# pyani-plus/pyani-plus

Measured on AMD Instinct MI355X. Metric: pairwise genome comparisons/sec (N x N ANI matrix), higher is better.
Workload: dtype u64

## Files before the change

### pyani_plus_amd/csrc/kmer_hash.hip

```cpp
#include <cstdlib>
#include <type_traits>
#include <utility>

#include "pa_internal.h"
#include "murmur_dev.h"

namespace {

using namespace pa_dev;

constexpr int kThreads = 256;
constexpr uint32_t kStageCap = 1024;

constexpr int pow2_floor(int k) { int c = 1; while (2 * c <= k) c *= 2; return c; }

__device__ __forceinline__ uint32_t find_genome(const uint32_t *__restrict__ genome_blk, uint32_t n, uint32_t blk) {
  uint32_t lo = 0, hi = n;
  while (hi - lo > 1) {
    uint32_t mid = (lo + hi) >> 1;
    if (genome_blk[mid] <= blk) lo = mid; else hi = mid;
  }
  return lo;
}

__device__ __forceinline__ void region_append(const CandSink &s, uint32_t g, uint64_t h) {
  const uint64_t slot = atomicAdd(&s.cursor[g], 1u);
  if (slot < s.region_off[g + 1] - s.region_off[g]) s.cand_hash[s.region_off[g] + slot] = h; else *s.overflow = 1u;
}

__device__ __forceinline__ void append_candidate(const CandSink &s, uint32_t g, uint64_t h) {
  if (s.region_off) {
    region_append(s, g, h);
  } else {
    const unsigned long long slot = atomicAdd(reinterpret_cast<unsigned long long *>(s.count), 1ULL);
    if (slot < s.cap) {
      s.cand_hash[slot] = h;
      s.cand_genome[slot] = g;
    }
  }
}

__device__ __forceinline__ void stage_candidate(const CandSink &s, uint64_t (&s_hash)[kStageCap], uint32_t (&s_blk)[kStageCap],
                                                uint32_t &s_n, uint32_t t, uint64_t h) {
  const uint32_t slot = atomicAdd(&s_n, 1u);
  if (slot < kStageCap) {
    s_hash[slot] = h;
    s_blk[slot] = t;
  } else if (s.region_off) {
    region_append(s, find_genome(s.genome_blk, s.n_genomes, t), h);
  } else {
    const unsigned long long g = atomicAdd(reinterpret_cast<unsigned long long *>(s.count), 1ULL);
    if (g < s.cap) {
      s.cand_hash[g] = h;
      s.cand_genome[g] = find_genome(s.genome_blk, s.n_genomes, t);
    }
  }
}

__device__ __forceinline__ void flush_staged(const CandSink &s, const uint64_t (&s_hash)[kStageCap], const uint32_t (&s_blk)[kStageCap],
                                             const uint32_t &s_n, unsigned long long &s_base, uint32_t blk0, uint32_t n_blocks64) {
  const uint32_t tid = threadIdx.x;
  __syncthreads();
  const uint32_t n = min(s_n, kStageCap);
  if (n == 0) return;
  if (s.region_off) {
    const uint32_t b0 = blk0 + blockIdx.x * kThreads;
    const uint32_t b1 = min(b0 + (uint32_t)kThreads, n_blocks64) - 1u;
    const uint32_t g0 = find_genome(s.genome_blk, s.n_genomes, b0);
    if (s.genome_blk[g0 + 1] > b1) {
      if (tid == 0) s_base = atomicAdd(&s.cursor[g0], n);
      __syncthreads();
      const uint64_t room = s.region_off[g0 + 1] - s.region_off[g0];
      uint64_t *__restrict__ dst = s.cand_hash + s.region_off[g0];
      for (uint32_t i = tid; i < n; i += kThreads) {
        const uint64_t slot = s_base + i;
        if (slot < room) dst[slot] = s_hash[i]; else *s.overflow = 1u;
      }
    } else {
      for (uint32_t i = tid; i < n; i += kThreads)
        region_append(s, find_genome(s.genome_blk, s.n_genomes, s_blk[i]), s_hash[i]);
    }
    return;
  }
  if (tid == 0) s_base = atomicAdd(reinterpret_cast<unsigned long long *>(s.count), (unsigned long long)n);
  __syncthreads();
  const unsigned long long base = s_base;
  for (uint32_t i = tid; i < n; i += kThreads) {
    const unsigned long long g = base + i;
    if (g < s.cap) {
      s.cand_hash[g] = s_hash[i];
      s.cand_genome[g] = find_genome(s.genome_blk, s.n_genomes, s_blk[i]);
    }
  }
}

__device__ __forceinline__ uint32_t rev_groups32(uint32_t x) {
  x = __builtin_bitreverse32(x);
  return ((x >> 1) & 0x55555555u) | ((x & 0x55555555u) << 1);
}

template <int K, bool LUT>
__global__ __launch_bounds__(kThreads) void kmer_hash_kernel(
    const uint4 *__restrict__ packed, const uint2 *__restrict__ mask, const uint64_t *__restrict__ dirty, uint32_t n_blocks64,
    const uint32_t *__restrict__ genome_blk, uint32_t n_genomes, uint64_t max_hash,
    uint64_t *__restrict__ cand_hash, uint32_t *__restrict__ cand_genome, uint64_t cap,
    unsigned long long *__restrict__ count, const uint64_t *__restrict__ region_off, uint32_t *__restrict__ cursor,
    uint32_t *__restrict__ overflow, uint32_t blk0) {
  static_assert(K >= 1 && K <= 32, "a k-mer is one 64-bit register pair");
  __shared__ uint64_t s_hash[kStageCap];
  __shared__ uint32_t s_blk[kStageCap];
  __shared__ uint32_t s_n;
  __shared__ unsigned long long s_base;
  constexpr int kWords = (K + 7) / 8;
  __shared__ uint64_t s_lo[LUT ? kWords : 1][256];
  __shared__ uint32_t s_hi[LUT ? kWords : 1][256];

  const uint32_t tid = threadIdx.x;
  const CandSink sink{cand_hash, cand_genome, cap, reinterpret_cast<uint64_t *>(count), region_off, cursor, overflow, genome_blk, n_genomes};
  const uint32_t max_hi = (uint32_t)(max_hash >> 32);
  const bool take_all = max_hi == 0xffffffffu;
  const uint32_t screen_hi = max_hi + 1u;
  if (tid == 0) s_n = 0;
  if constexpr (LUT) fill_first_products(s_lo, s_hi, tid, std::integral_constant<int, K>{});
  __syncthreads();

  const uint32_t t = blk0 + blockIdx.x * kThreads + tid;
  if (t < n_blocks64) {
    const uint4 cur = packed[t];
    uint2 pw = make_uint2(0u, 0u);
    if (t > 0) pw = reinterpret_cast<const uint2 *>(packed)[2 * (uint64_t)t - 1];
    uint32_t d1 = 0u, d2 = 0u;
    const uint32_t wave_blk = __builtin_amdgcn_readfirstlane(t & ~63u);
    const uint64_t dirty_word = dirty[wave_blk >> 6];
    if ((dirty_word >> (t & 63u)) & 1ull) {
      const uint2 m = mask[t];
      uint32_t d0 = t > 0 ? mask[t - 1].y : 0xffffffffu;
      d1 = m.x;
      d2 = m.y;
      int c = 1;
#pragma unroll
      for (; 2 * c <= K; c *= 2) {
        d2 |= alignbit(d2, d1, 32 - c);
        d1 |= alignbit(d1, d0, 32 - c);
        d0 |= d0 << c;
      }
      constexpr int cc = pow2_floor(K);
      constexpr int r = K - cc;
      if constexpr (r > 0) {
        d2 |= alignbit(d2, d1, 32 - r);
        d1 |= alignbit(d1, d0, 32 - r);
      }
    }
    const uint32_t bad[2] = {d1, d2};
    if ((d1 & d2) != 0xffffffffu) {
      constexpr uint64_t kMask = (K == 32) ? ~0ULL : ((1ULL << (2 * K)) - 1);
      constexpr uint32_t kMaskHi = (uint32_t)(kMask >> 32);
      uint32_t fw[8] = {pw.x, pw.y, cur.x, cur.y, cur.z, cur.w, 0u, 0u};
      uint32_t rw[6];
#pragma unroll
      for (int j = 0; j < 6; ++j) rw[j] = ~rev_groups32(fw[5 - j]);
      auto columns = [&](auto base_tag, int i_begin, int i_end) {
        constexpr int kBase = decltype(base_tag)::value;
#pragma unroll 1
        for (int i = i_begin; i < i_end; ++i) {
          constexpr int kOff = 33 - K;
          const uint32_t fo = 2u * (uint32_t)((i + kOff) & 15), ro = 30u - 2u * (uint32_t)i;
          uint32_t A[5], B[5];
#pragma unroll
          for (int j = 0; j < 5; ++j) {
            A[j] = alignbit(fw[kBase + j + 1], fw[kBase + j], fo);
            B[j] = alignbit(rw[j + 1], rw[j], ro);
          }
#pragma unroll
          for (int wi = 0; wi < 4; ++wi) {
            const uint32_t f_lo = A[wi], f_hi = A[wi + 1], r_lo = B[3 - wi], r_hi = B[4 - wi];
          const uint64_t f_lsb = u64_of(f_lo, f_hi) & kMask, r_lsb = u64_of(r_lo, r_hi) & kMask;
          const uint64_t fwd = __builtin_amdgcn_uicmpl(f_lsb, r_lsb, 37 );
          uint32_t clo, chi;
          asm("s_nop 1\n\tv_cndmask_b32_e64 %0, %1, %2, %3" : "=v"(clo) : "v"((uint32_t)r_lsb), "v"((uint32_t)f_lsb), "s"(fwd));
          asm("v_cndmask_b32_e64 %0, %1, %2, %3" : "=v"(chi) : "v"((uint32_t)(r_lsb >> 32)), "v"((uint32_t)(f_lsb >> 32)), "s"(fwd), "v"(clo));
          uint64_t P[4] = {0, 0, 0, 0};
#pragma unroll
          for (int j = 0; j < kWords; ++j) {
            const uint32_t src = j < 2 ? clo : chi;
            if constexpr (LUT) {
              P[j] = first_product(s_lo, s_hi, j, src);
            } else {
              const uint32_t glo = (src >> (16 * (j & 1))) & 0xffu, ghi = (src >> (16 * (j & 1) + 8)) & 0xffu;
              const uint64_t word = u64_of(ascii_group(glo, K - 8 * j), ascii_group(ghi, K - 8 * j - 4));
              P[j] = word * ((j & 1) ? kC2 : kC1);
            }
          }
          (void)kMaskHi;
          uint64_t U, V;
          murmur3_pre_last_mul<K>(P, U, V);
          if (passes_screen(U, V, take_all, screen_hi)) {
            const uint64_t h = last_mul_and_fold(U, V);
            if (h > max_hash || ((bad[wi >> 1] >> (16 * (wi & 1) + i)) & 1u)) continue;
            stage_candidate(sink, s_hash, s_blk, s_n, t, h);
          }
          }
        }
      };
      constexpr int kOff0 = 33 - K, kSplit = (kOff0 & 15) ? 16 - (kOff0 & 15) : 16;
      columns(std::integral_constant<int, (kOff0 >> 4)>{}, 0, kSplit);
      if constexpr (kSplit < 16) columns(std::integral_constant<int, (kOff0 >> 4) + 1>{}, kSplit, 16);
    }
  }
  flush_staged(sink, s_hash, s_blk, s_n, s_base, blk0, n_blocks64);
}

template <int K>
__global__ __launch_bounds__(kThreads) void kmer_hash_wide_kernel(
    const uint4 *__restrict__ packed, const uint2 *__restrict__ mask, const uint64_t *__restrict__ dirty, uint32_t n_blocks64,
    const uint32_t *__restrict__ genome_blk, uint32_t n_genomes, uint64_t max_hash,
    uint64_t *__restrict__ cand_hash, uint32_t *__restrict__ cand_genome, uint64_t cap,
    unsigned long long *__restrict__ count, const uint64_t *__restrict__ region_off, uint32_t *__restrict__ cursor,
    uint32_t *__restrict__ overflow, uint32_t blk0) {
  static_assert(K >= 33 && K <= 64, "k-mers of 65 to 128 bits");
  __shared__ uint64_t s_hash[kStageCap];
  __shared__ uint32_t s_blk[kStageCap];
  __shared__ uint32_t s_n;
  __shared__ unsigned long long s_base;
  constexpr int kWords = (K + 7) / 8;
  __shared__ uint64_t s_lo[kWords][256];
  __shared__ uint32_t s_hi[kWords][256];
  const uint32_t tid = threadIdx.x;
  const CandSink sink{cand_hash, cand_genome, cap, reinterpret_cast<uint64_t *>(count), region_off, cursor, overflow, genome_blk, n_genomes};
  const uint32_t max_hi = (uint32_t)(max_hash >> 32);
  const bool take_all = max_hi == 0xffffffffu;
  const uint32_t screen_hi = max_hi + 1u;
  if (tid == 0) s_n = 0;
  fill_first_products(s_lo, s_hi, tid, std::integral_constant<int, K>{});
  __syncthreads();

  const uint32_t t = blk0 + blockIdx.x * kThreads + tid;
  if (t < n_blocks64) {
    const uint4 cur = packed[t];
    const uint4 prev = t > 0 ? packed[t - 1] : make_uint4(0u, 0u, 0u, 0u);
    uint32_t d2 = 0u, d3 = 0u;
    const uint32_t wave_blk = __builtin_amdgcn_readfirstlane(t & ~63u);
    const uint64_t dirty_word = dirty[wave_blk >> 6];
    const uint64_t before = wave_blk ? dirty[(wave_blk >> 6) - 1] >> 63 : 1ull;
    const uint64_t dirty_or_prev = dirty_word | (dirty_word << 1) | before;
    if ((dirty_or_prev >> (t & 63u)) & 1ull) {
      const uint2 m = mask[t];
      uint32_t d0 = 0xffffffffu, d1 = 0xffffffffu;
      if (t > 0) { const uint2 mp = mask[t - 1]; d0 = mp.x; d1 = mp.y; }
      d2 = m.x;
      d3 = m.y;
#pragma unroll
      for (int c = 1; c <= 16; c *= 2) {
        d3 |= alignbit(d3, d2, 32 - c);
        d2 |= alignbit(d2, d1, 32 - c);
        d1 |= alignbit(d1, d0, 32 - c);
        d0 |= d0 << c;
      }
      if constexpr (K == 64) {
        d3 |= d2; d2 |= d1; d1 |= d0;
      } else {
        constexpr int r = K - 32;
        d3 |= alignbit(d3, d2, 32 - r);
        d2 |= alignbit(d2, d1, 32 - r);
        d1 |= alignbit(d1, d0, 32 - r);
      }
    }
    const uint32_t bad[2] = {d2, d3};
    if ((d2 & d3) != 0xffffffffu) {
      constexpr uint32_t kMask2 = (2 * K - 64 >= 32) ? 0xffffffffu : ((1u << (2 * K - 64)) - 1u);
      constexpr uint32_t kMask3 = (2 * K - 96 >= 32) ? 0xffffffffu : (2 * K - 96 <= 0 ? 0u : ((1u << ((2 * K - 96) & 31)) - 1u));
      const uint32_t fw[10] = {prev.x, prev.y, prev.z, prev.w, cur.x, cur.y, cur.z, cur.w, 0u, 0u};
      uint32_t rw[10];
#pragma unroll
      for (int j = 0; j < 10; ++j) rw[j] = ~rev_groups32(fw[9 - j]);
      auto columns = [&](auto base_tag, int i_begin, int i_end) {
        constexpr int kBase = decltype(base_tag)::value;
#pragma unroll 1
        for (int i = i_begin; i < i_end; ++i) {
          constexpr int kOff = 65 - K;
          const uint32_t fo = 2u * (uint32_t)((i + kOff) & 15), ro = 30u - 2u * (uint32_t)i;
          uint32_t A[7], B[7];
#pragma unroll
          for (int j = 0; j < 7; ++j) {
            A[j] = alignbit(fw[kBase + j + 1], fw[kBase + j], fo);
            B[j] = alignbit(rw[j + 3], rw[j + 2], ro);
          }
#pragma unroll
          for (int wi = 0; wi < 4; ++wi) {
            const uint32_t f0 = A[wi], f1 = A[wi + 1], f2 = A[wi + 2] & kMask2, f3 = A[wi + 3] & kMask3;
            const uint32_t r0 = B[3 - wi], r1 = B[4 - wi], r2 = B[5 - wi] & kMask2, r3 = B[6 - wi] & kMask3;
            const uint64_t lt_hi = __builtin_amdgcn_uicmpl(u64_of(f2, f3), u64_of(r2, r3), 36 );
            const uint64_t eq_hi = __builtin_amdgcn_uicmpl(u64_of(f2, f3), u64_of(r2, r3), 32 );
            const uint64_t le_lo = __builtin_amdgcn_uicmpl(u64_of(f0, f1), u64_of(r0, r1), 37 );
            const uint64_t fwd = lt_hi | (eq_hi & le_lo);
            uint32_t c0, c1, c2, c3;
            asm("s_nop 1\n\tv_cndmask_b32_e64 %0, %1, %2, %3" : "=v"(c0) : "v"(r0), "v"(f0), "s"(fwd));
            asm("v_cndmask_b32_e64 %0, %1, %2, %3" : "=v"(c1) : "v"(r1), "v"(f1), "s"(fwd), "v"(c0));
            asm("v_cndmask_b32_e64 %0, %1, %2, %3" : "=v"(c2) : "v"(r2), "v"(f2), "s"(fwd), "v"(c1));
            asm("v_cndmask_b32_e64 %0, %1, %2, %3" : "=v"(c3) : "v"(r3), "v"(f3), "s"(fwd), "v"(c2));
            const uint32_t cw[4] = {c0, c1, c2, c3};
            uint64_t P[8] = {0, 0, 0, 0, 0, 0, 0, 0};
#pragma unroll
            for (int j = 0; j < kWords; ++j) P[j] = first_product(s_lo, s_hi, j, cw[j >> 1]);
            uint64_t U, V;
            murmur3_pre_last_mul<K>(P, U, V);
            if (passes_screen(U, V, take_all, screen_hi)) {
              const uint64_t h = last_mul_and_fold(U, V);
              if (h > max_hash || ((bad[wi >> 1] >> (16 * (wi & 1) + i)) & 1u)) continue;
              stage_candidate(sink, s_hash, s_blk, s_n, t, h);
            }
          }
        }
      };
      constexpr int kOff0 = 65 - K, kSplit = (kOff0 & 15) ? 16 - (kOff0 & 15) : 16;
      columns(std::integral_constant<int, (kOff0 >> 4)>{}, 0, kSplit);
      if constexpr (kSplit < 16) columns(std::integral_constant<int, (kOff0 >> 4) + 1>{}, kSplit, 16);
    }
  }
  flush_staged(sink, s_hash, s_blk, s_n, s_base, blk0, n_blocks64);
}

constexpr int kLongIter = 32;
__global__ __launch_bounds__(kThreads) void kmer_hash_long_kernel(
    const uint32_t *__restrict__ packed, const uint32_t *__restrict__ mask, uint64_t pos0, uint64_t pos1, uint32_t k,
    const uint32_t *__restrict__ genome_blk, uint32_t n_genomes, uint64_t max_hash, uint64_t *__restrict__ cand_hash,
    uint32_t *__restrict__ cand_genome, uint64_t cap, unsigned long long *__restrict__ count,
    const uint64_t *__restrict__ region_off, uint32_t *__restrict__ cursor, uint32_t *__restrict__ overflow) {
  __shared__ uint64_t s_lo[8][256];
  __shared__ uint32_t s_hi[8][256];
  const uint32_t tid = threadIdx.x;
  const CandSink sink{cand_hash, cand_genome, cap, reinterpret_cast<uint64_t *>(count), region_off, cursor, overflow, genome_blk, n_genomes};
  const uint32_t n_words = (k + 7u) >> 3;
  const uint32_t max_hi = (uint32_t)(max_hash >> 32);
  const bool take_all = max_hi == 0xffffffffu;
  const uint32_t screen_hi = max_hi + 1u;
  fill_first_products(s_lo, s_hi, tid, k);
  __syncthreads();
  const uint64_t wg_first = pos0 + ((uint64_t)blockIdx.y * gridDim.x + blockIdx.x) * (uint64_t)(kThreads * kLongIter);
#pragma unroll 1
  for (int it = 0; it < kLongIter; ++it) {
  const uint64_t e = wg_first + (uint64_t)it * kThreads + tid;
  if (e >= pos1 || e + 1 < k) continue;
  const uint64_t a = e + 1 - k;
  {
    const uint64_t m0 = a >> 5, m_last = e >> 5;
    const uint32_t sm = (uint32_t)(a & 31u);
    const uint32_t w0 = mask[m0], w1 = m0 + 1 <= m_last ? mask[m0 + 1] : 0u, w2 = m0 + 2 <= m_last ? mask[m0 + 2] : 0u;
    const uint32_t b0 = alignbit(w1, w0, sm), b1 = alignbit(w2, w1, sm);
    const uint32_t top = k == 64 ? 0xffffffffu : ((1u << (k - 32u)) - 1u);
    if (b0 | (b1 & top)) continue;
  }
  uint32_t F[4], R[4];
  {
    const uint64_t p0 = a >> 4, p_last = e >> 4;
    const uint32_t sp = 2u * (uint32_t)(a & 15u);
    uint32_t w[5];
#pragma unroll
    for (int i = 0; i < 5; ++i) w[i] = p0 + i <= p_last ? packed[p0 + i] : 0u;
#pragma unroll
    for (int i = 0; i < 4; ++i) F[i] = alignbit(w[i + 1], w[i], sp);
    const uint32_t used = 2u * k - 64u;
    if (used < 32u) { F[2] &= (1u << used) - 1u; F[3] = 0u; }
    else if (used < 64u) F[3] &= (1u << (used - 32u)) - 1u;
    const uint32_t C[6] = {~rev_groups32(F[3]), ~rev_groups32(F[2]), ~rev_groups32(F[1]), ~rev_groups32(F[0]), 0u, 0u};
    const uint32_t s = 128u - 2u * k, ws = s >> 5, bs = s & 31u;
#pragma unroll
    for (int i = 0; i < 4; ++i) R[i] = ws ? alignbit(C[i + 2], C[i + 1], bs) : alignbit(C[i + 1], C[i], bs);
    if (used < 32u) { R[2] &= (1u << used) - 1u; R[3] = 0u; }
    else if (used < 64u) R[3] &= (1u << (used - 32u)) - 1u;
  }
  const uint64_t f_hi = u64_of(F[2], F[3]), f_lo = u64_of(F[0], F[1]), r_hi = u64_of(R[2], R[3]), r_lo = u64_of(R[0], R[1]);
  const bool fwd = f_hi < r_hi || (f_hi == r_hi && f_lo <= r_lo);
  uint32_t c[4];
#pragma unroll
  for (int i = 0; i < 4; ++i) c[i] = fwd ? F[i] : R[i];
  uint64_t P[8] = {0, 0, 0, 0, 0, 0, 0, 0};
#pragma unroll
  for (uint32_t j = 0; j < 8; ++j) {
    if (j >= n_words) break;
    P[j] = first_product(s_lo, s_hi, j, c[j >> 1]);
  }
  uint64_t U, V;
  murmur3_pre_last_mul_rt(P, k, U, V);
  if (!passes_screen(U, V, take_all, screen_hi)) continue;
  const uint64_t h = last_mul_and_fold(U, V);
  if (h > max_hash) continue;
  append_candidate(sink, find_genome(genome_blk, n_genomes, (uint32_t)(e >> 6)), h);
  }
}

template <class Kernel>
int launch_blocks(pa_ctx *c, const char *name, Kernel kernel, const KmerHashArgs &a) {
  const ArenaView &v = a.arena;
  const CandSink &s = a.sink;
  return pa_launch(c, name, kernel, false, ceil_div(v.n_blocks64 - a.blk0, kThreads), kThreads, 0, a.stream,
                   reinterpret_cast<const uint4 *>(v.packed), reinterpret_cast<const uint2 *>(v.mask), v.dirty,
                   (uint32_t)v.n_blocks64, s.genome_blk, s.n_genomes, a.max_hash, s.cand_hash, s.cand_genome, s.cap,
                   reinterpret_cast<unsigned long long *>(s.count), s.region_off, s.cursor, s.overflow, (uint32_t)a.blk0);
}

template <int K>
int launch_k(pa_ctx *c, const KmerHashArgs &a) {
  if constexpr (K > 32) {
    return launch_blocks(c, "kmer_hash_wide_kernel", kmer_hash_wide_kernel<K>, a);
  } else {
    if constexpr (K == 31) {
      static const bool arithmetic = [] {
        const char *v = PA_TOOL_ENV("PA_KMER_VARIANT");
        return v && v[0] == '0';
      }();
      if (arithmetic) return launch_blocks(c, "kmer_hash_kernel<31, false>", kmer_hash_kernel<K, false>, a);
    }
    return launch_blocks(c, "kmer_hash_kernel", kmer_hash_kernel<K, true>, a);
  }
}

}

int pa_launch_kmer_hash(pa_ctx *c, const KmerHashArgs &a) {
  const uint64_t n_blocks64 = a.arena.n_blocks64;
  PA_REQUIRE(n_blocks64 < (1ULL << 32), "arena too large: %llu blocks of 64 bases", (unsigned long long)n_blocks64);
  if (n_blocks64 <= a.blk0) return PA_OK;
  const char *long_form = PA_TOOL_ENV("PA_KMER_LONG");
  if (a.k > 32 && a.k <= 64 && long_form && long_form[0] == 'p') {
    const CandSink &s = a.sink;
    const uint64_t pos0 = a.blk0 * 64, pos1 = n_blocks64 * 64;
    const uint64_t per_wg = (uint64_t)kThreads * kLongIter;
    const uint64_t n_wg = (pos1 - pos0 + per_wg - 1) / per_wg;
    const uint32_t gx = (uint32_t)std::min<uint64_t>(n_wg, 1u << 20), gy = (uint32_t)((n_wg + gx - 1) / gx);
    PA_REQUIRE(gy <= 65535u, "arena too large for one launch of the long k-mer kernel: %llu positions", (unsigned long long)(pos1 - pos0));
    return PA_LAUNCH_ON(c, a.stream, kmer_hash_long_kernel, LaunchDim(gx, gy), kThreads, 0, a.arena.packed, a.arena.mask, pos0, pos1, a.k,
                        s.genome_blk, s.n_genomes, a.max_hash, s.cand_hash, s.cand_genome, s.cap,
                        reinterpret_cast<unsigned long long *>(s.count), s.region_off, s.cursor, s.overflow);
  }
  PA_REQUIRE((a.blk0 & 63u) == 0, "k-mer hash launch must start at a multiple of 64 blocks, not %llu", (unsigned long long)a.blk0);
  int status = PA_E_INVALID;
  if (!dispatch_value(a.k, value_list<1, 64>{}, [&](auto k) { status = launch_k<k()>(c, a); })) pa_set_error("k=%u outside [1,64]", a.k);
  return status;
}
```

### pyani_plus_amd/csrc/murmur_dev.h

```cpp
#pragma once

#include <hip/hip_runtime.h>

#include <cstdint>

namespace pa_dev {

__device__ __forceinline__ uint32_t alignbit(uint32_t hi, uint32_t lo, uint32_t sh) {
  return __builtin_amdgcn_alignbit(hi, lo, sh);
}

__device__ __forceinline__ uint32_t ascii4(uint32_t b8) {
  uint32_t u = (b8 | (b8 << 12)) & 0x000F000Fu;
  uint32_t v = (u | (u << 6)) & 0x03030303u;
  return __builtin_amdgcn_perm(0u, 0x54474341u, v);
}

__device__ __forceinline__ uint64_t u64_of(uint32_t lo, uint32_t hi) { return ((uint64_t)hi << 32) | lo; }

__device__ __forceinline__ uint64_t rotl64(uint64_t x, int r) {
  const uint32_t lo = (uint32_t)x, hi = (uint32_t)(x >> 32);
  if (r == 32) return u64_of(hi, lo);
  if (r < 32) return u64_of(alignbit(lo, hi, 32 - r), alignbit(hi, lo, 32 - r));
  return u64_of(alignbit(hi, lo, 64 - r), alignbit(lo, hi, 64 - r));
}

__device__ __forceinline__ uint64_t fmix64(uint64_t k) {
  k ^= k >> 33;
  k *= 0xff51afd7ed558ccdULL;
  k ^= k >> 33;
  k *= 0xc4ceb9fe1a85ec53ULL;
  k ^= k >> 33;
  return k;
}

constexpr uint64_t kC1 = 0x87c37b91114253d5ULL, kC2 = 0x4cf5ad432745937fULL;

__device__ __forceinline__ uint64_t times5_plus(uint64_t h, uint64_t c) {
  uint64_t t;
  asm("v_lshl_add_u64 %0, %1, 2, %1" : "=v"(t) : "v"(h));
  return t + c;
}

constexpr uint64_t kF1 = 0xff51afd7ed558ccdULL, kF2 = 0xc4ceb9fe1a85ec53ULL;

template <int K, int N>
__device__ __forceinline__ void murmur3_pre_last_mul(const uint64_t (&P)[N], uint64_t &U, uint64_t &V) {
  static_assert(N >= (K + 7) / 8, "one first product per 8-byte word of the k-mer");
  uint64_t h1 = 42, h2 = 42;
  constexpr int nblocks = K / 16;
  constexpr int tail = K % 16;
#pragma unroll
  for (int i = 0; i < nblocks; ++i) {
    const uint64_t k1 = rotl64(P[2 * i], 31) * kC2;
    h1 ^= k1;
    if (i == 0) {
      h1 = times5_plus(rotl64(h1, 27), 5ULL * 42ULL + 0x52dce729ULL);
    } else {
      h1 = rotl64(h1, 27) + h2;
      h1 = times5_plus(h1, 0x52dce729ULL);
    }
    const uint64_t k2 = rotl64(P[2 * i + 1], 33) * kC1;
    h2 ^= k2;
    h2 = rotl64(h2, 31) + h1;
    h2 = times5_plus(h2, 0x38495ab5ULL);
  }
  if constexpr (tail > 8) h2 ^= rotl64(P[2 * nblocks + 1], 33) * kC1;
  if constexpr (tail > 0) h1 ^= rotl64(P[2 * nblocks], 31) * kC2;
  h1 ^= (uint64_t)K; h2 ^= (uint64_t)K;
  h1 += h2; h2 += h1;
  h1 ^= h1 >> 33; h1 *= kF1; h1 ^= h1 >> 33;
  h2 ^= h2 >> 33; h2 *= kF1; h2 ^= h2 >> 33;
  U = h1;
  V = h2;
}

__device__ __forceinline__ void murmur3_pre_last_mul_rt(const uint64_t (&P)[8], uint32_t k, uint64_t &U, uint64_t &V) {
  uint64_t h1 = 42, h2 = 42;
  const uint32_t nblocks = k >> 4, tail = k & 15u;
#pragma unroll
  for (uint32_t i = 0; i < 4; ++i) {
    if (i >= nblocks) break;
    h1 ^= rotl64(P[2 * i], 31) * kC2;
    h1 = rotl64(h1, 27) + h2;
    h1 = times5_plus(h1, 0x52dce729ULL);
    h2 ^= rotl64(P[2 * i + 1], 33) * kC1;
    h2 = rotl64(h2, 31) + h1;
    h2 = times5_plus(h2, 0x38495ab5ULL);
  }
  uint64_t t1 = 0, t2 = 0;
#pragma unroll
  for (uint32_t i = 0; i < 4; ++i)
    if (i == nblocks) { t1 = P[2 * i]; t2 = P[2 * i + 1]; }
  if (tail > 8) h2 ^= rotl64(t2, 33) * kC1;
  if (tail > 0) h1 ^= rotl64(t1, 31) * kC2;
  h1 ^= (uint64_t)k;
  h2 ^= (uint64_t)k;
  h1 += h2;
  h2 += h1;
  h1 ^= h1 >> 33; h1 *= kF1; h1 ^= h1 >> 33;
  h2 ^= h2 >> 33; h2 *= kF1; h2 ^= h2 >> 33;
  U = h1;
  V = h2;
}

__device__ __forceinline__ uint32_t last_mul_high_sum_plus1(uint64_t U, uint64_t V) {
  constexpr uint32_t c0 = (uint32_t)kF2, c1 = (uint32_t)(kF2 >> 32);
  const uint32_t u0 = (uint32_t)U, u1 = (uint32_t)(U >> 32), v0 = (uint32_t)V, v1 = (uint32_t)(V >> 32);
  return (__umulhi(u0, c0) + __umulhi(v0, c0) + 1u) + ((u0 + v0) * c1 + (u1 + v1) * c0);
}

__device__ __forceinline__ bool passes_screen(uint64_t U, uint64_t V, bool take_all, uint32_t screen_hi) {
  return take_all || last_mul_high_sum_plus1(U, V) <= screen_hi;
}
__device__ __forceinline__ uint64_t last_mul_and_fold(uint64_t U, uint64_t V) {
  const uint64_t X = U * kF2, Y = V * kF2;
  return (X ^ (X >> 33)) + (Y ^ (Y >> 33));
}

template <int K, int N>
__device__ __forceinline__ uint64_t murmur3_from_products(const uint64_t (&P)[N]) {
  uint64_t U, V;
  murmur3_pre_last_mul<K, N>(P, U, V);
  return last_mul_and_fold(U, V);
}

__device__ __forceinline__ uint32_t ascii_group(uint32_t b8, int nv) {
  const uint32_t a = ascii4(b8);
  return nv >= 4 ? a : (nv <= 0 ? 0u : (a & ((1u << (8 * nv)) - 1u)));
}

template <int W, class KInt>
__device__ __forceinline__ void fill_first_products(uint64_t (&s_lo)[W][256], uint32_t (&s_hi)[W][256], uint32_t tid, KInt k_) {
  const int k = (int)k_;
  const int n_words = (int)(((uint32_t)k + 7u) >> 3);
#pragma unroll
  for (int j = 0; j < n_words; ++j) {
    const uint64_t cj = (j & 1) ? kC2 : kC1;
    s_lo[j][tid] = (uint64_t)ascii_group(tid, k - 8 * j) * cj;
    s_hi[j][tid] = (uint32_t)((uint64_t)ascii_group(tid, k - 8 * j - 4) * cj);
  }
}

template <int W>
__device__ __forceinline__ uint64_t first_product(const uint64_t (&s_lo)[W][256], const uint32_t (&s_hi)[W][256], uint32_t j, uint32_t src) {
  const uint32_t glo = (src >> (16u * (j & 1u))) & 0xffu, ghi = (src >> (16u * (j & 1u) + 8u)) & 0xffu;
  const uint64_t lo = s_lo[j][glo];
  return u64_of((uint32_t)lo, (uint32_t)(lo >> 32) + s_hi[j][ghi]);
}

}
```

Measured before the change: 79.71 million.

## Precompute second MurmurHash3 products in LDS tables for k-mer hashing

```diff
diff --git a/pyani_plus_amd/csrc/kmer_hash.hip b/pyani_plus_amd/csrc/kmer_hash.hip
--- a/pyani_plus_amd/csrc/kmer_hash.hip
+++ b/pyani_plus_amd/csrc/kmer_hash.hip
@@ -11,6 +11,7 @@
 
 constexpr int kThreads = 256;
 constexpr uint32_t kStageCap = 1024;
+constexpr uint32_t kStageCapSecond = 512;
 
 constexpr int pow2_floor(int k) { int c = 1; while (2 * c <= k) c *= 2; return c; }
 
@@ -40,10 +41,11 @@
   }
 }
 
-__device__ __forceinline__ void stage_candidate(const CandSink &s, uint64_t (&s_hash)[kStageCap], uint32_t (&s_blk)[kStageCap],
+template <uint32_t Cap>
+__device__ __forceinline__ void stage_candidate(const CandSink &s, uint64_t (&s_hash)[Cap], uint32_t (&s_blk)[Cap],
                                                 uint32_t &s_n, uint32_t t, uint64_t h) {
   const uint32_t slot = atomicAdd(&s_n, 1u);
-  if (slot < kStageCap) {
+  if (slot < Cap) {
     s_hash[slot] = h;
     s_blk[slot] = t;
   } else if (s.region_off) {
@@ -57,11 +59,12 @@
   }
 }
 
-__device__ __forceinline__ void flush_staged(const CandSink &s, const uint64_t (&s_hash)[kStageCap], const uint32_t (&s_blk)[kStageCap],
+template <uint32_t Cap>
+__device__ __forceinline__ void flush_staged(const CandSink &s, const uint64_t (&s_hash)[Cap], const uint32_t (&s_blk)[Cap],
                                              const uint32_t &s_n, unsigned long long &s_base, uint32_t blk0, uint32_t n_blocks64) {
   const uint32_t tid = threadIdx.x;
   __syncthreads();
-  const uint32_t n = min(s_n, kStageCap);
+  const uint32_t n = min(s_n, Cap);
   if (n == 0) return;
   if (s.region_off) {
     const uint32_t b0 = blk0 + blockIdx.x * kThreads;
@@ -99,7 +102,8 @@
   return ((x >> 1) & 0x55555555u) | ((x & 0x55555555u) << 1);
 }
 
-template <int K, bool LUT>
+enum WordForm { kArithmetic = 0, kFirstTables = 1, kSecondTables = 2 };
+template <int K, WordForm FORM>
 __global__ __launch_bounds__(kThreads) void kmer_hash_kernel(
     const uint4 *__restrict__ packed, const uint2 *__restrict__ mask, const uint64_t *__restrict__ dirty, uint32_t n_blocks64,
     const uint32_t *__restrict__ genome_blk, uint32_t n_genomes, uint64_t max_hash,
@@ -107,13 +111,15 @@
     unsigned long long *__restrict__ count, const uint64_t *__restrict__ region_off, uint32_t *__restrict__ cursor,
     uint32_t *__restrict__ overflow, uint32_t blk0) {
   static_assert(K >= 1 && K <= 32, "a k-mer is one 64-bit register pair");
-  __shared__ uint64_t s_hash[kStageCap];
-  __shared__ uint32_t s_blk[kStageCap];
+  constexpr uint32_t kCap = FORM == kSecondTables ? kStageCapSecond : kStageCap;
+  __shared__ uint64_t s_hash[kCap];
+  __shared__ uint32_t s_blk[kCap];
   __shared__ uint32_t s_n;
   __shared__ unsigned long long s_base;
   constexpr int kWords = (K + 7) / 8;
-  __shared__ uint64_t s_lo[LUT ? kWords : 1][256];
-  __shared__ uint32_t s_hi[LUT ? kWords : 1][256];
+  __shared__ uint64_t s_lo[FORM == kFirstTables ? kWords : 1][256];
+  __shared__ uint4 s_w[FORM == kSecondTables ? kWords : 1][256];
+  __shared__ uint32_t s_hi[FORM != kArithmetic ? kWords : 1][256];
 
   const uint32_t tid = threadIdx.x;
   const CandSink sink{cand_hash, cand_genome, cap, reinterpret_cast<uint64_t *>(count), region_off, cursor, overflow, genome_blk, n_genomes};
@@ -121,7 +127,8 @@
   const bool take_all = max_hi == 0xffffffffu;
   const uint32_t screen_hi = max_hi + 1u;
   if (tid == 0) s_n = 0;
-  if constexpr (LUT) fill_first_products(s_lo, s_hi, tid, std::integral_constant<int, K>{});
+  if constexpr (FORM == kFirstTables) fill_first_products(s_lo, s_hi, tid, std::integral_constant<int, K>{});
+  if constexpr (FORM == kSecondTables) fill_second_products(s_w, s_hi, tid, K);
   __syncthreads();
 
   const uint32_t t = blk0 + blockIdx.x * kThreads + tid;
@@ -183,7 +190,9 @@
 #pragma unroll
           for (int j = 0; j < kWords; ++j) {
             const uint32_t src = j < 2 ? clo : chi;
-            if constexpr (LUT) {
+            if constexpr (FORM == kSecondTables) {
+              P[j] = second_product(s_w, s_hi, j, src);
+            } else if constexpr (FORM == kFirstTables) {
               P[j] = first_product(s_lo, s_hi, j, src);
             } else {
               const uint32_t glo = (src >> (16 * (j & 1))) & 0xffu, ghi = (src >> (16 * (j & 1) + 8)) & 0xffu;
@@ -193,7 +202,7 @@
           }
           (void)kMaskHi;
           uint64_t U, V;
-          murmur3_pre_last_mul<K>(P, U, V);
+          if constexpr (FORM == kSecondTables) murmur3_pre_last_mul_of_seconds<K>(P, U, V); else murmur3_pre_last_mul<K>(P, U, V);
           if (passes_screen(U, V, take_all, screen_hi)) {
             const uint64_t h = last_mul_and_fold(U, V);
             if (h > max_hash || ((bad[wi >> 1] >> (16 * (wi & 1) + i)) & 1u)) continue;
@@ -404,14 +413,14 @@
   if constexpr (K > 32) {
     return launch_blocks(c, "kmer_hash_wide_kernel", kmer_hash_wide_kernel<K>, a);
   } else {
+#ifdef PA_TOOLS
     if constexpr (K == 31) {
-      static const bool arithmetic = [] {
-        const char *v = PA_TOOL_ENV("PA_KMER_VARIANT");
-        return v && v[0] == '0';
-      }();
-      if (arithmetic) return launch_blocks(c, "kmer_hash_kernel<31, false>", kmer_hash_kernel<K, false>, a);
-    }
-    return launch_blocks(c, "kmer_hash_kernel", kmer_hash_kernel<K, true>, a);
+      const char *v = PA_TOOL_ENV("PA_KMER_VARIANT");
+      if (v && v[0] == '0') return launch_blocks(c, "kmer_hash_kernel<31, kArithmetic>", kmer_hash_kernel<K, kArithmetic>, a);
+      if (v && v[0] == '1') return launch_blocks(c, "kmer_hash_kernel<31, kFirstTables>", kmer_hash_kernel<K, kFirstTables>, a);
+    }
+#endif
+    return launch_blocks(c, "kmer_hash_kernel", kmer_hash_kernel<K, kSecondTables>, a);
   }
 }
 
diff --git a/pyani_plus_amd/csrc/murmur_dev.h b/pyani_plus_amd/csrc/murmur_dev.h
--- a/pyani_plus_amd/csrc/murmur_dev.h
+++ b/pyani_plus_amd/csrc/murmur_dev.h
@@ -3,17 +3,13 @@
 #include <hip/hip_runtime.h>
 
 #include <cstdint>
+
+#include "murmur_words.h"
 
 namespace pa_dev {
 
 __device__ __forceinline__ uint32_t alignbit(uint32_t hi, uint32_t lo, uint32_t sh) {
   return __builtin_amdgcn_alignbit(hi, lo, sh);
-}
-
-__device__ __forceinline__ uint32_t ascii4(uint32_t b8) {
-  uint32_t u = (b8 | (b8 << 12)) & 0x000F000Fu;
-  uint32_t v = (u | (u << 6)) & 0x03030303u;
-  return __builtin_amdgcn_perm(0u, 0x54474341u, v);
 }
 
 __device__ __forceinline__ uint64_t u64_of(uint32_t lo, uint32_t hi) { return ((uint64_t)hi << 32) | lo; }
@@ -34,7 +30,6 @@
   return k;
 }
 
-constexpr uint64_t kC1 = 0x87c37b91114253d5ULL, kC2 = 0x4cf5ad432745937fULL;
 
 __device__ __forceinline__ uint64_t times5_plus(uint64_t h, uint64_t c) {
   uint64_t t;
@@ -75,6 +70,36 @@
   V = h2;
 }
 
+template <int K, int N>
+__device__ __forceinline__ void murmur3_pre_last_mul_of_seconds(const uint64_t (&Kw)[N], uint64_t &U, uint64_t &V) {
+  static_assert(N >= (K + 7) / 8, "one second product per 8-byte word of the k-mer");
+  uint64_t h1 = 42, h2 = 42;
+  constexpr int nblocks = K / 16;
+  constexpr int tail = K % 16;
+#pragma unroll
+  for (int i = 0; i < nblocks; ++i) {
+    h1 ^= Kw[2 * i];
+    if (i == 0) {
+      h1 = times5_plus(rotl64(h1, 27), 5ULL * 42ULL + 0x52dce729ULL);
+    } else {
+      h1 = rotl64(h1, 27) + h2;
+      h1 = times5_plus(h1, 0x52dce729ULL);
+    }
+    h2 ^= Kw[2 * i + 1];
+    uint64_t r2 = rotl64(h2, 31);
+    asm("" : "+v"(r2));
+    h2 = times5_plus(r2 + h1, 0x38495ab5ULL);
+  }
+  if constexpr (tail > 8) h2 ^= Kw[2 * nblocks + 1];
+  if constexpr (tail > 0) h1 ^= Kw[2 * nblocks];
+  h1 ^= (uint64_t)K; h2 ^= (uint64_t)K;
+  h1 += h2; h2 += h1;
+  h1 ^= h1 >> 33; h1 *= kF1; h1 ^= h1 >> 33;
+  h2 ^= h2 >> 33; h2 *= kF1; h2 ^= h2 >> 33;
+  U = h1;
+  V = h2;
+}
+
 __device__ __forceinline__ void murmur3_pre_last_mul_rt(const uint64_t (&P)[8], uint32_t k, uint64_t &U, uint64_t &V) {
   uint64_t h1 = 42, h2 = 42;
   const uint32_t nblocks = k >> 4, tail = k & 15u;
@@ -125,11 +150,6 @@
   return last_mul_and_fold(U, V);
 }
 
-__device__ __forceinline__ uint32_t ascii_group(uint32_t b8, int nv) {
-  const uint32_t a = ascii4(b8);
-  return nv >= 4 ? a : (nv <= 0 ? 0u : (a & ((1u << (8 * nv)) - 1u)));
-}
-
 template <int W, class KInt>
 __device__ __forceinline__ void fill_first_products(uint64_t (&s_lo)[W][256], uint32_t (&s_hi)[W][256], uint32_t tid, KInt k_) {
   const int k = (int)k_;
@@ -149,4 +169,37 @@
   return u64_of((uint32_t)lo, (uint32_t)(lo >> 32) + s_hi[j][ghi]);
 }
 
-}
+template <int W>
+__device__ __forceinline__ void fill_second_products(uint4 (&s_w)[W][256], uint32_t (&s_b)[W][256], uint32_t tid, int k) {
+#pragma unroll
+  for (int j = 0; j < W; ++j) {
+    const WordLoEntry e = word_lo_entry(j, k, tid);
+    s_w[j][tid] = make_uint4(e.t_lo, e.t_hi, e.a_hi, e.pad);
+    s_b[j][tid] = word_hi_entry(j, k, tid);
+  }
+}
+
+template <uint32_t SH>
+__device__ __forceinline__ uint32_t byte_offset(uint32_t src, uint32_t byte) {
+  uint32_t r;
+  const uint32_t sh = SH;
+  switch (byte) {
+    case 0: asm("v_lshlrev_b32_sdwa %0, %1, %2 dst_sel:DWORD dst_unused:UNUSED_PAD src0_sel:DWORD src1_sel:BYTE_0" : "=v"(r) : "v"(sh), "v"(src)); break;
+    case 1: asm("v_lshlrev_b32_sdwa %0, %1, %2 dst_sel:DWORD dst_unused:UNUSED_PAD src0_sel:DWORD src1_sel:BYTE_1" : "=v"(r) : "v"(sh), "v"(src)); break;
+    case 2: asm("v_lshlrev_b32_sdwa %0, %1, %2 dst_sel:DWORD dst_unused:UNUSED_PAD src0_sel:DWORD src1_sel:BYTE_2" : "=v"(r) : "v"(sh), "v"(src)); break;
+    default: asm("v_lshlrev_b32_sdwa %0, %1, %2 dst_sel:DWORD dst_unused:UNUSED_PAD src0_sel:DWORD src1_sel:BYTE_3" : "=v"(r) : "v"(sh), "v"(src)); break;
+  }
+  return r;
+}
+
+template <int W>
+__device__ __forceinline__ uint64_t second_product(const uint4 (&s_w)[W][256], const uint32_t (&s_b)[W][256], int j, uint32_t src) {
+  const uint32_t off_w = byte_offset<4>(src, 2u * (j & 1)), off_b = byte_offset<2>(src, 2u * (j & 1) + 1u);
+  typedef uint32_t u32x4 __attribute__((ext_vector_type(4)));
+  u32x4 e = *reinterpret_cast<const u32x4 *>(reinterpret_cast<const char *>(&s_w[j][0]) + off_w);
+  asm("" : "+v"(e));
+  const uint32_t b = *reinterpret_cast<const uint32_t *>(reinterpret_cast<const char *>(&s_b[j][0]) + off_b);
+  return second_product_of(j, e.x, e.y, e.z, b);
+}
+
+}
diff --git a/pyani_plus_amd/csrc/murmur_words.h b/pyani_plus_amd/csrc/murmur_words.h
--- /dev/null
+++ b/pyani_plus_amd/csrc/murmur_words.h
@@ -0,0 +1,66 @@
+#pragma once
+
+#include <cstdint>
+
+#if defined(__HIPCC__)
+#include <hip/hip_runtime.h>
+#define PA_WORDS_FN __host__ __device__ __forceinline__
+#else
+#define PA_WORDS_FN inline
+#endif
+
+namespace pa_dev {
+
+constexpr uint64_t kC1 = 0x87c37b91114253d5ULL, kC2 = 0x4cf5ad432745937fULL;
+
+PA_WORDS_FN uint32_t ascii4(uint32_t b8) {
+#if defined(__HIP_DEVICE_COMPILE__)
+  uint32_t u = (b8 | (b8 << 12)) & 0x000F000Fu;
+  uint32_t v = (u | (u << 6)) & 0x03030303u;
+  return __builtin_amdgcn_perm(0u, 0x54474341u, v);
+#else
+  uint32_t a = 0;
+  for (int i = 0; i < 4; ++i) a |= ((0x54474341u >> (8 * ((b8 >> (2 * i)) & 3u))) & 0xffu) << (8 * i);
+  return a;
+#endif
+}
+
+PA_WORDS_FN uint32_t ascii_group(uint32_t b8, int nv) {
+  const uint32_t a = ascii4(b8);
+  return nv >= 4 ? a : (nv <= 0 ? 0u : (a & ((1u << (8 * nv)) - 1u)));
+}
+
+PA_WORDS_FN constexpr uint64_t word_c_first(int j) { return (j & 1) ? kC2 : kC1; }
+PA_WORDS_FN constexpr uint64_t word_c_second(int j) { return (j & 1) ? kC1 : kC2; }
+
+struct WordLoEntry {
+  uint32_t t_lo, t_hi, a_hi, pad;
+};
+
+PA_WORDS_FN WordLoEntry word_lo_entry(int j, int k, uint32_t g) {
+  const uint64_t a = (uint64_t)ascii_group(g, k - 8 * j) * word_c_first(j);
+  const uint32_t a_lo = (uint32_t)a;
+  const uint64_t cb = word_c_second(j);
+  const uint64_t t = (j & 1) ? (((uint64_t)a_lo << 33) + (a_lo >> 31)) * cb : ((uint64_t)a_lo << 31) * cb;
+  return WordLoEntry{(uint32_t)t, (uint32_t)(t >> 32), (uint32_t)(a >> 32), 0u};
+}
+
+PA_WORDS_FN uint32_t word_hi_entry(int j, int k, uint32_t g) {
+  return (uint32_t)((uint64_t)ascii_group(g, k - 8 * j - 4) * word_c_first(j));
+}
+
+PA_WORDS_FN uint64_t second_product_of(int j, uint32_t t_lo, uint32_t t_hi, uint32_t a_hi, uint32_t b) {
+  const uint32_t s = a_hi + b;
+  const uint64_t t = ((uint64_t)t_hi << 32) | t_lo;
+  if (j & 1) {
+    const uint64_t c = word_c_second(j) << 1;
+    const uint64_t m = (uint64_t)s * (uint32_t)c + t;
+    return ((uint64_t)((uint32_t)(m >> 32) + s * (uint32_t)(c >> 32)) << 32) | (uint32_t)m;
+  }
+  const uint64_t c = word_c_second(j);
+  const uint32_t x = s >> 1;
+  const uint64_t m = (uint64_t)x * (uint32_t)c + t;
+  return ((uint64_t)((uint32_t)(m >> 32) + (x * (uint32_t)(c >> 32) + (s << 31))) << 32) | (uint32_t)m;
+}
+
+}
```

Result: faster. 87.29 million (median of 6 runs) (+9.5%).
